# hvak/visual-underwater-slam

Measured on AMD Instinct MI355X. Metric: ORB detect+match frames/sec, higher is better.
Workload: dtype u8

## Files before the change

visual-underwater-slam_amd/csrc/detect.hip:

```cpp
#include "frontend_common.h"
#include "../../include/vus_tiled.h"

namespace {

#ifndef VUS_FAST_WPE
#define VUS_FAST_WPE 1
#endif
#ifndef VUS_FAST_LDS_PAD
#define VUS_FAST_LDS_PAD 0
#endif
#ifdef VUS_FAST_EXIT_AFTER
#define VUS_FAST_EXIT(N) do { if (VUS_FAST_EXIT_AFTER == (N)) return; } while (0)
#else
#define VUS_FAST_EXIT(N)
#endif
#ifdef VUS_FAST_DEBUG_COUNT
__device__ unsigned long long g_fast_dbg[4];
extern "C" int vus_debug_fast_counters(unsigned long long* out, int reset) {
  if (hipMemcpyFromSymbol(out, HIP_SYMBOL(g_fast_dbg), sizeof(g_fast_dbg)) != hipSuccess) return -1;
  if (reset) { unsigned long long z[4] = {0, 0, 0, 0}; if (hipMemcpyToSymbol(HIP_SYMBOL(g_fast_dbg), z, sizeof(z)) != hipSuccess) return -1; }
  return 0;
}
#endif

constexpr int TW = VUS_FAST_TILE_W;
constexpr int TH = VUS_FAST_TILE_H;
constexpr int NTHREADS = 256;
constexpr int IMG_ROWS = TH + 8;
constexpr int IMG_DW = (TW + 16) / 4;
constexpr int SC_ROWS = TH + 2;
constexpr int SC_DW = (TW + 8) / 4;
constexpr int STRIPS = TW / 4;

__device__ __forceinline__ int min3i(int a, int b, int c) { return min(min(a, b), c); }
__device__ __forceinline__ int max3i(int a, int b, int c) { return max(max(a, b), c); }
__device__ __forceinline__ int byte_of(uint32_t w, int i) { return (int)((w >> (8 * i)) & 0xFFu); }

__device__ __forceinline__ int fast_score_bytes(const uint8_t* c, int rb) {
  constexpr int DX[16] = {0, 1, 2, 3, 3, 3, 2, 1, 0, -1, -2, -3, -3, -3, -2, -1};
  constexpr int DY[16] = {-3, -3, -2, -1, 0, 1, 2, 3, 3, 3, 2, 1, 0, -1, -2, -3};
  const int p = c[0];
  int d[16];
#pragma unroll
  for (int k = 0; k < 16; ++k) d[k] = (int)c[DY[k] * rb + DX[k]] - p;
  int mn3[16], mx3[16];
#pragma unroll
  for (int k = 0; k < 16; ++k) {
    mn3[k] = min3i(d[k], d[(k + 1) & 15], d[(k + 2) & 15]);
    mx3[k] = max3i(d[k], d[(k + 1) & 15], d[(k + 2) & 15]);
  }
  int best_bright = -(1 << 20), best_dark = 1 << 20;
#pragma unroll
  for (int k = 0; k < 16; ++k) {
    best_bright = max(best_bright, min3i(mn3[k], mn3[(k + 3) & 15], mn3[(k + 6) & 15]));
    best_dark = min(best_dark, max3i(mx3[k], mx3[(k + 3) & 15], mx3[(k + 6) & 15]));
  }
  return max(best_bright, -best_dark) - 1;
}

constexpr int VUS_CAND_REGIONS = 8;
struct BlurMfmaTable {
  uint64_t h[64];
  uint64_t v[2][64];
};
constexpr BlurMfmaTable make_blur_mfma_table() {
  constexpr int BW[7] = {18, 33, 49, 56, 49, 33, 18};
  BlurMfmaTable t{};
  for (int l = 0; l < 64; ++l) {
    const int g = l >> 4, m = l & 15;
    for (int sl = 0; sl < 8; ++sl) {
      const int d = 8 * g + sl - m - 5;
      if (d >= 0 && d <= 6) t.h[l] |= (uint64_t)BW[d] << (8 * sl);
      const int hrow = sl < 4 ? 4 * g + sl : 16 + 4 * g + (sl - 4);
      for (int nb = 0; nb < 2; ++nb) {
        const int dv = hrow - (16 * nb + m + 1);
        if (dv >= 0 && dv <= 6) t.v[nb][l] |= (uint64_t)BW[dv] << (8 * sl);
      }
    }
  }
  return t;
}
__device__ __attribute__((aligned(16))) const BlurMfmaTable g_blur_mfma_table = make_blur_mfma_table();
typedef int v4i32_t __attribute__((ext_vector_type(4)));

template <bool TILED = false>
__device__ __forceinline__ void blur_tile_mfma(const uint32_t* s_img, uint8_t* __restrict__ blur_out, int n, int H, int W,
                                               int x0, int y0, int tid, int j_first, int j_step) {
  static_assert(IMG_ROWS == 32 && TW % 16 == 0 && (IMG_DW * 4) % 8 == 0, "blur_tile_mfma: K = the 32 staged rows");
  const int l = tid & 63, g = l >> 4, m = l & 15;
  const long bh = (long)g_blur_mfma_table.h[l];
  const long bv[2] = {(long)g_blur_mfma_table.v[0][l], (long)g_blur_mfma_table.v[1][l]};
  const uint8_t* img8 = reinterpret_cast<const uint8_t*>(s_img);
  constexpr unsigned long long SIGN = 0x8080808080808080ull;
  const int j_end = TILED ? min(TW / 16, (W - x0) / 16) : TW / 16;
  bool row_ok[2] = {false, false};
  uint32_t tiled_off[2] = {0u, 0u};
  uint8_t* const tiled_plane = blur_out + (size_t)n * H * W;
  if (TILED) {
    j_first = __builtin_amdgcn_readfirstlane(j_first);
#pragma unroll
    for (int nb = 0; nb < 2; ++nb) {
      const int ly = 16 * nb + m;
      row_ok[nb] = ly < TH && y0 + ly < H;
      tiled_off[nb] = vus_tiled_offset(y0 + ly, x0 + 4 * g, W);
    }
  }
#pragma unroll 1
  for (int j = j_first; j < j_end; j += j_step) {
    v4i32_t ch[2];
#pragma unroll
    for (int mb = 0; mb < 2; ++mb) {
      const unsigned long long a =
          *reinterpret_cast<const unsigned long long*>(img8 + (16 * mb + m) * (IMG_DW * 4) + 16 * j + 8 * g) ^ SIGN;
      const v4i32_t c0 = {32768, 32768, 32768, 32768};
      ch[mb] = __builtin_amdgcn_mfma_i32_16x16x32_i8((long)a, bh, c0, 0, 0, 0);
    }
    uint32_t lo[2], hi[2];
#pragma unroll
    for (int mb = 0; mb < 2; ++mb) {
      const uint32_t t0 = __builtin_amdgcn_perm((uint32_t)ch[mb][1], (uint32_t)ch[mb][0], 0x05010400u);
      const uint32_t t1 = __builtin_amdgcn_perm((uint32_t)ch[mb][3], (uint32_t)ch[mb][2], 0x05010400u);
      lo[mb] = __builtin_amdgcn_perm(t1, t0, 0x05040100u);
      hi[mb] = __builtin_amdgcn_perm(t1, t0, 0x07060302u);
    }
    const long a_lo = (long)((((unsigned long long)lo[1] << 32) | lo[0]) ^ SIGN);
    const long a_hi = (long)((((unsigned long long)hi[1] << 32) | hi[0]) ^ SIGN);
#pragma unroll
    for (int nb = 0; nb < 2; ++nb) {
      const v4i32_t ci = {32768, 32768, 32768, 32768};
      const v4i32_t cl = {65536, 65536, 65536, 65536};
      const v4i32_t chi = __builtin_amdgcn_mfma_i32_16x16x32_i8(a_hi, bv[nb], ci, 0, 0, 0);
      const v4i32_t clo = __builtin_amdgcn_mfma_i32_16x16x32_i8(a_lo, bv[nb], cl, 0, 0, 0);
      uint32_t q[4];
#pragma unroll
      for (int r = 0; r < 4; ++r) q[r] = ((uint32_t)chi[r] << 8) + (uint32_t)clo[r];
      const uint32_t v = __builtin_amdgcn_perm(q[1], q[0], 0x0c0c0602u) | __builtin_amdgcn_perm(q[3], q[2], 0x06020c0cu);
      const int ly = 16 * nb + m, gy = y0 + ly, gx = x0 + 16 * j + 4 * g;
      if (TILED) {
        if (row_ok[nb]) __builtin_memcpy(tiled_plane + (tiled_off[nb] + (uint32_t)(VUS_TILE_BW * VUS_TILE_BH * j)), &v, 4);
      } else if (ly < TH && gy < H) {
        uint8_t* o = blur_out + ((size_t)n * H + gy) * W + gx;
        if (gx + 3 < W) {
          __builtin_memcpy(o, &v, 4);
        } else {
#pragma unroll
          for (int e = 0; e < 4; ++e)
            if (gx + e < W) o[e] = (uint8_t)(v >> (8 * e));
        }
      }
    }
  }
}

template <bool WRITE_SCORE, bool DETECT, bool BLUR, bool HIST = false, bool REGIONS = false, bool TILED = false>
__device__ __forceinline__ void fast_tile_body(
    const uint8_t* __restrict__ img, int H, int W, int pitch, int thr, int border,
    uint8_t* __restrict__ score_out, uint8_t* __restrict__ blur_out,
    uint32_t* __restrict__ cand_keys, int cand_cap, int* __restrict__ cand_count, int* __restrict__ hist,
    int n, int tile, int tiles_x, uint8_t* __restrict__ raw_out = nullptr) {
  static_assert(IMG_ROWS == 32, "the smoothing (blur_tile_mfma) takes the 32 staged rows as its K");
  constexpr bool SCORES = WRITE_SCORE || DETECT;
  constexpr bool LATE_BLUR = BLUR && DETECT && !HIST;
  static_assert(!TILED || LATE_BLUR, "the block-tiled planes are written by the late-smoothing detection launch");

  __shared__ __attribute__((aligned(8))) uint32_t s_img[IMG_ROWS * IMG_DW];
  __shared__ uint32_t s_score[SCORES ? SC_ROWS * SC_DW : 1];
  constexpr int AUX_DW = SCORES ? (IMG_ROWS * IMG_DW + SC_ROWS * SC_DW + 1) / 2 : 2;
  __shared__ uint32_t s_aux[AUX_DW];
  uint16_t* const s_mm = reinterpret_cast<uint16_t*>(s_aux);
  uint16_t* const s_strip = s_mm + IMG_ROWS * IMG_DW;
  __shared__ uint16_t s_work[SCORES ? SC_ROWS * SC_DW * 4 : 2];
  __shared__ int s_nstrip;
  __shared__ int s_cnt, s_base, s_nwork;
  static_assert(IMG_ROWS * IMG_DW >= TW * TH / 4, "candidate list must fit in the image tile");
  static_assert(!LATE_BLUR || AUX_DW >= TW * TH / 4, "candidate list must fit in the strip tables' buffer");
  uint32_t* const s_keys = LATE_BLUR ? s_aux : s_img;

  const int tid = threadIdx.x;
  const int x0 = (tile % tiles_x) * TW, y0 = (tile / tiles_x) * TH;
  const uint8_t* im = img + (size_t)n * H * pitch;

  {
    constexpr int RPP = NTHREADS / IMG_DW;
    const int col = tid % IMG_DW, r0 = tid / IMG_DW;
    const int gx = x0 - 8 + 4 * col;
    const bool fast = gx >= 0 && gx + 3 < W;
    const bool inside = x0 >= 8 && x0 + TW + 8 <= W && y0 >= 4 && y0 + TH + 4 <= H;
    if (r0 < RPP) {
      constexpr int NP = (IMG_ROWS + RPP - 1) / RPP;
      constexpr int LASTP = IMG_ROWS - (NP - 1) * RPP;
      uint32_t v[NP];
      if (inside) {
        const uint32_t off0 = (uint32_t)((y0 - 4 + r0) * pitch + gx);
        const uint32_t step = (uint32_t)(RPP * pitch);
#pragma unroll
        for (int k = 0; k < NP - 1; ++k) __builtin_memcpy(&v[k], im + (off0 + (uint32_t)k * step), 4);
        v[NP - 1] = 0u;
        if (r0 < LASTP) __builtin_memcpy(&v[NP - 1], im + (off0 + (uint32_t)(NP - 1) * step), 4);
      } else {
        const uint8_t* rp[NP];
#pragma unroll
        for (int k = 0; k < NP; ++k) rp[k] = im + (size_t)clampi(y0 - 4 + min(r0 + RPP * k, IMG_ROWS - 1), 0, H - 1) * pitch;
        if (fast) {
#pragma unroll
          for (int k = 0; k < NP; ++k) __builtin_memcpy(&v[k], rp[k] + gx, 4);
        } else {
          const int c0 = clampi(gx, 0, W - 1), c1 = clampi(gx + 1, 0, W - 1), c2 = clampi(gx + 2, 0, W - 1),
                    c3 = clampi(gx + 3, 0, W - 1);
          uint8_t q[NP][4];
#pragma unroll
          for (int k = 0; k < NP; ++k) { q[k][0] = rp[k][c0]; q[k][1] = rp[k][c1]; q[k][2] = rp[k][c2]; q[k][3] = rp[k][c3]; }
#pragma unroll
          for (int k = 0; k < NP; ++k)
            v[k] = (uint32_t)q[k][0] | ((uint32_t)q[k][1] << 8) | ((uint32_t)q[k][2] << 16) | ((uint32_t)q[k][3] << 24);
        }
      }
#pragma unroll
      for (int k = 0; k < NP; ++k) {
        const int row = r0 + RPP * k;
        if (row < IMG_ROWS) {
          s_img[row * IMG_DW + col] = v[k];
          if (SCORES) {
            const int b0 = byte_of(v[k], 0), b1 = byte_of(v[k], 1), b2 = byte_of(v[k], 2), b3 = byte_of(v[k], 3);
            s_mm[row * IMG_DW + col] = (uint16_t)(min(min(b0, b1), min(b2, b3)) | (max(max(b0, b1), max(b2, b3)) << 8));
          }
        }
      }
    }
  }
  if (tid == 0) { s_cnt = 0; s_nwork = 0; s_nstrip = 0; }
  __syncthreads();
  VUS_FAST_EXIT(1);

  if (SCORES) {
    static_assert(STRIPS == 32 && (TH * STRIPS) % NTHREADS == 0, "pass 1a: thread = (row tid >> 5, strip tid & 31)");
    constexpr int S_RPP = NTHREADS / STRIPS;
    constexpr int NMAIN = TH / S_RPP;
    constexpr int NIT = NMAIN + 1;
    static_assert(SC_DW + TH <= 64 && SC_ROWS == TH + 2 && SC_DW == STRIPS + 2, "pass 1a: the ring pass is a row and a column per wave");
    auto strip_test = [&](int sr, int ss, int ci) -> bool {
      const int gy = y0 - 1 + sr, gx = x0 - 4 + 4 * ss;
      if (!((uint32_t)gx < (uint32_t)max(W - 3, 0) && (uint32_t)(gy - 3) < (uint32_t)max(H - 6, 0))) return false;
      const uint8_t* mm8 = reinterpret_cast<const uint8_t*>(s_mm) + 2 * ci;
      const int ma_lo = mm8[0], ma_hi = mm8[1], pmin = mm8[2], pmax = mm8[3], mc_lo = mm8[4], mc_hi = mm8[5];
      const int mn_lo = mm8[2 - 6 * IMG_DW], mn_hi = mm8[3 - 6 * IMG_DW], ms_lo = mm8[2 + 6 * IMG_DW], ms_hi = mm8[3 + 6 * IMG_DW];
      const uint32_t b = s_img[ci + 1];
      const int b0 = byte_of(b, 0), b3 = byte_of(b, 3);
      const int hi = min(max(mn_hi, ms_hi), max3i(ma_hi, mc_hi, max(b0, b3)));
      const int lo = max(min(mn_lo, ms_lo), min3i(ma_lo, mc_lo, min(b0, b3)));
      return hi > pmin + thr || lo < pmax - thr;
    };
    const int sr0 = 1 + (tid >> 5), ss0 = 1 + (tid & 31);
    unsigned long long bal[NIT];
    bool pass[NIT];
    int ent[NIT];
#pragma unroll
    for (int it = 0; it < NMAIN; ++it) {
      const int sr = sr0 + it * S_RPP;
      pass[it] = strip_test(sr, ss0, (sr0 + 3) * IMG_DW + ss0 + it * S_RPP * IMG_DW);
      s_score[sr0 * SC_DW + ss0 + it * S_RPP * SC_DW] = 0u;
      ent[it] = sr * SC_DW + ss0;
      bal[it] = __ballot(pass[it]);
    }
    pass[NMAIN] = false;
    ent[NMAIN] = 0;
    bal[NMAIN] = 0ull;
    const int wv = __builtin_amdgcn_readfirstlane(tid >> 6);
    if (wv < 2) {
      const int l = tid & 63;
      const bool is_row = l < SC_DW;
      const int sr = is_row ? wv * (SC_ROWS - 1) : l - (SC_DW - 1);
      const int ss = is_row ? l : wv * (SC_DW - 1);
      if (l < SC_DW + TH) {
        pass[NMAIN] = strip_test(sr, ss, (sr + 3) * IMG_DW + ss);
        s_score[sr * SC_DW + ss] = 0u;
        ent[NMAIN] = sr * SC_DW + ss;
      }
      bal[NMAIN] = __ballot(pass[NMAIN]);
    }
    int total = 0;
#pragma unroll
    for (int it = 0; it < NIT; ++it) total += __popcll(bal[it]);
    if (total > 0) {
      int base = 0;
      if ((tid & 63) == 0) base = atomicAdd(&s_nstrip, total);
      base = __builtin_amdgcn_readfirstlane(base);
#pragma unroll
      for (int it = 0; it < NIT; ++it) {
        if (pass[it])
          s_strip[base + __builtin_amdgcn_mbcnt_hi((uint32_t)(bal[it] >> 32), __builtin_amdgcn_mbcnt_lo((uint32_t)bal[it], 0))] =
              (uint16_t)ent[it];
        base += __popcll(bal[it]);
      }
    }
    __syncthreads();
    VUS_FAST_EXIT(2);
    const int nstrip = s_nstrip;
#ifdef VUS_FAST_DEBUG_COUNT
    if (tid == 0 && BLUR) { atomicAdd(&g_fast_dbg[0], 1ull); atomicAdd(&g_fast_dbg[1], (unsigned long long)nstrip); }
#endif
    for (int j0 = 0; j0 < nstrip; j0 += NTHREADS) {
      const int j = j0 + tid;
      int mask = 0, idx = 0;
      if (j < nstrip) {
        idx = s_strip[j];
        const int sr = idx / SC_DW, ss = idx - sr * SC_DW;
        const int gx = x0 - 4 + 4 * ss;
        const uint32_t* cp = &s_img[(sr + 3) * IMG_DW + ss];
        const uint32_t a = cp[0], b = cp[1], c = cp[2];
        const uint32_t nn = s_img[sr * IMG_DW + ss + 1], so = s_img[(sr + 6) * IMG_DW + ss + 1];
        const uint32_t wv = __builtin_amdgcn_alignbyte(b, a, 1);
        const uint32_t ev = __builtin_amdgcn_alignbyte(c, b, 3);
        const uint32_t* up = &s_img[(sr + 1) * IMG_DW + ss];
        const uint32_t* dn = &s_img[(sr + 5) * IMG_DW + ss];
        const uint32_t nev = __builtin_amdgcn_alignbyte(up[2], up[1], 2), nwv = __builtin_amdgcn_alignbyte(up[1], up[0], 2);
        const uint32_t sev = __builtin_amdgcn_alignbyte(dn[2], dn[1], 2), swv = __builtin_amdgcn_alignbyte(dn[1], dn[0], 2);
#pragma unroll
        for (int e = 0; e < 4; ++e) {
          const int p = byte_of(b, e);
          const int n_ = byte_of(nn, e), s_ = byte_of(so, e), w_ = byte_of(wv, e), e_ = byte_of(ev, e);
          int hi = min(max(n_, s_), max(e_, w_)), lo = max(min(n_, s_), min(e_, w_));
          const int ne = byte_of(nev, e), sw = byte_of(swv, e), se = byte_of(sev, e), nw = byte_of(nwv, e);
          hi = min3i(hi, max(ne, sw), max(se, nw));
          lo = max3i(lo, min(ne, sw), min(se, nw));
          mask |= (hi > p + thr || lo < p - thr) ? (1 << e) : 0;
        }
        if (gx < 3 || gx + 3 >= W - 3) {
#pragma unroll
          for (int e = 0; e < 4; ++e)
            if (gx + e < 3 || gx + e >= W - 3) mask &= ~(1 << e);
        }
      }
      const int cnt = __popc(mask);
      int incl = cnt;
      incl += __builtin_amdgcn_update_dpp(0, incl, 0x111, 0xf, 0xf, true);
      incl += __builtin_amdgcn_update_dpp(0, incl, 0x112, 0xf, 0xf, true);
      incl += __builtin_amdgcn_update_dpp(0, incl, 0x114, 0xf, 0xe, true);
      incl += __builtin_amdgcn_update_dpp(0, incl, 0x118, 0xf, 0xc, true);
      incl += __builtin_amdgcn_update_dpp(0, incl, 0x142, 0xa, 0xf, true);
      incl += __builtin_amdgcn_update_dpp(0, incl, 0x143, 0xc, 0xf, true);
      const int total = __builtin_amdgcn_readlane(incl, 63);
      int base = 0;
      if ((tid & 63) == 0 && total > 0) base = atomicAdd(&s_nwork, total);
      base = __builtin_amdgcn_readfirstlane(base);
      int pos = base + incl - cnt;
#pragma unroll
      for (int e = 0; e < 4; ++e)
        if (mask & (1 << e)) s_work[pos++] = (uint16_t)(idx * 4 + e);
    }
  }
#ifdef VUS_FAST_DEBUG_COUNT
  __syncthreads();
  if (tid == 0 && BLUR && SCORES) atomicAdd(&g_fast_dbg[2], (unsigned long long)s_nwork);
#endif
  VUS_FAST_EXIT(3);
  if (BLUR && !LATE_BLUR) blur_tile_mfma(s_img, blur_out, n, H, W, x0, y0, tid, tid >> 6, NTHREADS / 64);
  __syncthreads();
  VUS_FAST_EXIT(4);

  if (SCORES) {
    const int nwork = s_nwork;
    uint8_t* score8 = reinterpret_cast<uint8_t*>(s_score);
    for (int j = tid; j < nwork; j += NTHREADS) {
      const int ent = s_work[j];
      const int idx = ent >> 2, e = ent & 3;
      const int sr = idx / SC_DW, ss = idx - sr * SC_DW;
      const int sc = fast_score_bytes(reinterpret_cast<const uint8_t*>(s_img) + (sr + 3) * (4 * IMG_DW) + 4 * (ss + 1) + e, 4 * IMG_DW);
      if (sc >= thr) score8[ent] = (uint8_t)sc;
    }
    __syncthreads();
  }
  VUS_FAST_EXIT(5);

  if (WRITE_SCORE) {
    for (int idx = tid; idx < TH * STRIPS; idx += NTHREADS) {
      const int ly = idx / STRIPS, ls = idx - ly * STRIPS;
      const int gy = y0 + ly, gx = x0 + 4 * ls;
      const uint32_t v = s_score[(ly + 1) * SC_DW + ls + 1];
      if (gy < H) {
        uint8_t* o = score_out + ((size_t)n * H + gy) * W + gx;
#pragma unroll
        for (int e = 0; e < 4; ++e)
          if (gx + e < W) o[e] = (uint8_t)(v >> (8 * e));
      }
    }
  }
  if (DETECT) {
    const int nwork = s_nwork;
    const uint8_t* score8 = reinterpret_cast<const uint8_t*>(s_score);
    for (int j = tid; j < nwork; j += NTHREADS) {
      const int ent = s_work[j];
      const int s = score8[ent];
      if (s == 0) continue;
      const int sr = ent / (4 * SC_DW), sx = ent - sr * (4 * SC_DW);
      const int ly = sr - 1, lx = sx - 4;
      if (ly < 0 || ly >= TH || lx < 0 || lx >= TW) continue;
      const int gy = y0 + ly, gx = x0 + lx;
      if (gy < border || gy >= H - border || gx < border || gx >= W - border) continue;
      const uint8_t* c = score8 + ent;
      constexpr int RB = 4 * SC_DW;
      const int m = max3i(max3i(c[-RB - 1], c[-RB], c[-RB + 1]), max((int)c[-1], (int)c[1]), max3i(c[RB - 1], c[RB], c[RB + 1]));
      if (s > m) {
        if (HIST) {
          atomicAdd(&hist[256 * n + s], 1);
        } else {
          const int p = atomicAdd(&s_cnt, 1);
          s_keys[p] = ((uint32_t)(255 - s) << VUS_KEY_POS_BITS) | (uint32_t)(gy * W + gx);
        }
      }
    }
    if (!HIST) {
      __syncthreads();
      const int cnt = s_cnt;
      const int rcap = cand_cap / VUS_CAND_REGIONS;
      uint32_t* const list = cand_keys + (size_t)n * cand_cap + (REGIONS ? (size_t)(tile & (VUS_CAND_REGIONS - 1)) * rcap : 0);
      int* const counter = REGIONS ? reinterpret_cast<int*>(list) : &cand_count[n];
      if (LATE_BLUR) {
        const bool leader = tid == NTHREADS - 64 && cnt > 0;
        int base = 0;
        if (leader) base = atomicAdd(counter, cnt);
        if (TILED && tid >= NTHREADS - 64) {
          const uint8_t* s8 = reinterpret_cast<const uint8_t*>(s_img);
          uint8_t* const ro = raw_out + (size_t)n * H * W;
          for (int i = tid - (NTHREADS - 64); i < TH * (TW / 16); i += 64) {
            const int ly = i / (TW / 16), cb = i - ly * (TW / 16);
            const int gy = y0 + ly, gx = x0 + 16 * cb;
            if (gy < H && gx < W) {
              const uint8_t* sp = s8 + (ly + 4) * (4 * IMG_DW) + 8 + 16 * cb;
              const uint2 a = *reinterpret_cast<const uint2*>(sp), b = *reinterpret_cast<const uint2*>(sp + 8);
              *reinterpret_cast<uint4*>(ro + vus_tiled_offset(gy, gx, W)) = make_uint4(a.x, a.y, b.x, b.y);
            }
          }
        }
        if (leader) s_base = base;
        if (tid < NTHREADS - 64) blur_tile_mfma<TILED>(s_img, blur_out, n, H, W, x0, y0, tid, tid >> 6, NTHREADS / 64 - 1);
      } else {
        if (tid == 0 && cnt > 0) s_base = atomicAdd(counter, cnt);
      }
      __syncthreads();
      if (cnt > 0) {
        const int base = s_base + (REGIONS ? 1 : 0), lim = REGIONS ? rcap : cand_cap;
        for (int i = tid; i < cnt; i += NTHREADS)
          if (base + i < lim) list[base + i] = s_keys[i];
      }
    }
  }
}

template <bool WRITE_SCORE, bool DETECT, bool BLUR, bool REGIONS = false>
__global__ __launch_bounds__(NTHREADS, VUS_FAST_WPE) void fast_tile_kernel(
    const uint8_t* __restrict__ img, int H, int W, int pitch, int thr, const int* __restrict__ thr_img, int border,
    uint8_t* __restrict__ score_out, uint8_t* __restrict__ blur_out,
    uint32_t* __restrict__ cand_keys, int cand_cap, int* __restrict__ cand_count, int n_img, int tiles_x,
    int tiles_per_img) {
  const int xcd = blockIdx.x & 7, slot = blockIdx.x >> 3;
  const int n = (slot / tiles_per_img) * 8 + xcd;
  if (n >= n_img) return;
  const int tile = slot - (slot / tiles_per_img) * tiles_per_img;
  fast_tile_body<WRITE_SCORE, DETECT, BLUR, false, REGIONS>(img, H, W, pitch, thr_img ? thr_img[n] : thr, border, score_out, blur_out,
                                                            cand_keys, cand_cap, cand_count, nullptr, n, tile, tiles_x);
}

template <bool REGIONS>
__global__ __launch_bounds__(NTHREADS, VUS_FAST_WPE) void fast_tile_tiled_kernel(
    const uint8_t* __restrict__ img, int H, int W, int pitch, const int* __restrict__ thr_img, int border,
    uint8_t* __restrict__ blur_out, uint8_t* __restrict__ raw_out, uint32_t* __restrict__ cand_keys, int cand_cap,
    int* __restrict__ cand_count, int n_img, int tiles_x, int tiles_per_img) {
  const int xcd = blockIdx.x & 7, slot = blockIdx.x >> 3;
  const int n = (slot / tiles_per_img) * 8 + xcd;
  if (n >= n_img) return;
  const int tile = slot - (slot / tiles_per_img) * tiles_per_img;
  fast_tile_body<false, true, true, false, REGIONS, true>(img, H, W, pitch, thr_img[n], border, nullptr, blur_out, cand_keys,
                                                          cand_cap, cand_count, nullptr, n, tile, tiles_x, raw_out);
}

__global__ void cand_region_zero_kernel(uint32_t* __restrict__ cand_keys, int cand_cap, int n_img) {
  const int t = blockIdx.x * blockDim.x + threadIdx.x;
  if (t < n_img * VUS_CAND_REGIONS)
    cand_keys[(size_t)(t / VUS_CAND_REGIONS) * cand_cap + (size_t)(t % VUS_CAND_REGIONS) * (cand_cap / VUS_CAND_REGIONS)] = 0u;
}

__global__ __launch_bounds__(256) void cand_region_merge_kernel(uint32_t* __restrict__ cand_keys, int cand_cap, int* __restrict__ cand_count) {
  __shared__ int s_c[VUS_CAND_REGIONS];
  const int n = blockIdx.x, tid = threadIdx.x;
  const int rcap = cand_cap / VUS_CAND_REGIONS;
  uint32_t* row = cand_keys + (size_t)n * cand_cap;
  if (tid < VUS_CAND_REGIONS) s_c[tid] = (int)row[(size_t)tid * rcap];
  __syncthreads();
  int off = 0;
  long long all = 0;
  bool over = false;
  for (int r = 0; r < VUS_CAND_REGIONS; ++r) {
    const int c = s_c[r], m = min(c, rcap - 1);
    all += c;
    over |= c > rcap - 1;
    const uint32_t* src = row + (size_t)r * rcap + 1;
    for (int i0 = 0; i0 < m; i0 += 256) {
      const int i = i0 + tid;
      const uint32_t v = i < m ? src[i] : 0u;
      __syncthreads();
      if (i < m) row[off + i] = v;
      __syncthreads();
    }
    off += m;
  }
  if (over)
    for (int i = off + tid; i < cand_cap; i += 256) row[i] = VUS_KEY_INVALID;
  if (tid == 0) cand_count[n] = over ? (int)max(all, (long long)cand_cap + 1) : off;
}

__global__ __launch_bounds__(NTHREADS, VUS_FAST_WPE) void fast_sample_kernel(const uint8_t* __restrict__ img, int H, int W, int pitch,
                                                               int thr, int border, int* __restrict__ hist, int n_img,
                                                               int tiles_x, int tiles_per_img, int stride, int n_sampled) {
  const int xcd = blockIdx.x & 7, slot = blockIdx.x >> 3;
  const int n = (slot / n_sampled) * 8 + xcd;
  if (n >= n_img) return;
  const int tile = (slot - (slot / n_sampled) * n_sampled) * stride + stride / 2;
  if (tile >= tiles_per_img) return;
  fast_tile_body<false, true, false, true>(img, H, W, pitch, thr, border, nullptr, nullptr, nullptr, 0, nullptr, hist, n, tile, tiles_x);
}

__global__ __launch_bounds__(256) void fast_pick_threshold_kernel(const int* __restrict__ hist, int n_img, int thr, int floor, int max_kp,
                                                                  long long n_tiles, long long n_sampled, int num, int den,
                                                                  int* __restrict__ thr_img) {
  const int n = blockIdx.x * 4 + (threadIdx.x >> 6), lane = threadIdx.x & 63;
  if (n >= n_img) return;
  const int4 h = reinterpret_cast<const int4*>(hist + 256 * (size_t)n)[lane];
  const int hv[4] = {h.x, h.y, h.z, lane == 63 ? 0 : h.w};
  int above = hv[0] + hv[1] + hv[2] + hv[3];
  int incl = above;
#pragma unroll
  for (int d = 1; d < 64; d <<= 1) {
    const int o = __shfl_down(incl, d);
    if (lane + d < 64) incl += o;
  }
  above = incl - above;
  const long long need = (long long)max_kp * n_sampled * num;
  long long run = above;
  int best = -1;
#pragma unroll
  for (int q = 3; q >= 0; --q) {
    run += hv[q];
    const int t = 4 * lane + q;
    if (best < 0 && t > floor && t <= 254 && run * n_tiles * den >= need) best = t;
  }
#pragma unroll
  for (int d = 32; d >= 1; d >>= 1) best = max(best, __shfl_xor(best, d));
  if (lane == 0) thr_img[n] = best > floor ? best : thr;
}

__global__ __launch_bounds__(1024) void fast_retry_list_kernel(const int* __restrict__ thr_img, int thr, int max_kp, int cand_cap,
                                                               int n_img, int* __restrict__ cand_count,
                                                               int* __restrict__ retry_list, int* __restrict__ retry_count) {
  __shared__ int s_n;
  if (threadIdx.x == 0) s_n = 0;
  __syncthreads();
  for (int n = threadIdx.x; n < n_img; n += 1024)
    if ((thr_img[n] > thr && cand_count[n] < max_kp) || cand_count[n] > cand_cap) {
      retry_list[atomicAdd(&s_n, 1)] = n;
      cand_count[n] = 0;
    }
  __syncthreads();
  if (threadIdx.x == 0) retry_count[0] = s_n;
}

__global__ __launch_bounds__(NTHREADS, VUS_FAST_WPE) void fast_retry_kernel(const uint8_t* __restrict__ img, int H, int W, int pitch, int thr,
                                                              int border, uint32_t* __restrict__ cand_keys, int cand_cap,
                                                              int* __restrict__ cand_count, const int* __restrict__ retry_list,
                                                              const int* __restrict__ retry_count, int tiles_x, int tiles_per_img) {
  const long long items = (long long)retry_count[0] * tiles_per_img;
  for (long long it = blockIdx.x; it < items; it += gridDim.x) {
    const int n = retry_list[it / tiles_per_img], tile = (int)(it % tiles_per_img);
    fast_tile_body<false, true, false>(img, H, W, pitch, thr, border, nullptr, nullptr, cand_keys, cand_cap, cand_count, nullptr, n,
                                       tile, tiles_x);
    __syncthreads();
  }
}

struct TileGrid {
  unsigned blocks;
  int tiles_x, tiles_per_img;
};
TileGrid tile_grid(int n_img, int H, int W) {
  const int tx = (W + TW - 1) / TW, ty = (H + TH - 1) / TH;
  return TileGrid{(unsigned)(((n_img + 7) / 8) * 8 * tx * ty), tx, tx * ty};
}

}

extern "C" int vus_fast_score(const uint8_t* img, int n_img, int H, int W, int pitch, int thr,
                              uint8_t* score_out, void* stream) {
  if (int rc = check_image_args(img, n_img, H, W, pitch)) return rc;
  VUS_REQUIRE(score_out != nullptr, "score_out is null");
  VUS_REQUIRE(thr >= 1 && thr <= 254, "thr=%d out of range [1, 254]", thr);
  if (n_img == 0) return VUS_OK;
  const TileGrid g = tile_grid(n_img, H, W);
  fast_tile_kernel<true, false, false><<<g.blocks, NTHREADS, 0, vus::as_stream(stream)>>>(
      img, H, W, pitch, thr, nullptr, 0, score_out, nullptr, nullptr, 0, nullptr, n_img, g.tiles_x, g.tiles_per_img);
  VUS_CHECK_LAUNCH("fast_score");
  return VUS_OK;
}

extern "C" int vus_blur7(const uint8_t* img, int n_img, int H, int W, int pitch, uint8_t* out, void* stream) {
  if (int rc = check_image_args(img, n_img, H, W, pitch)) return rc;
  VUS_REQUIRE(out != nullptr, "out is null");
  if (n_img == 0) return VUS_OK;
  const TileGrid g = tile_grid(n_img, H, W);
  fast_tile_kernel<false, false, true><<<g.blocks, NTHREADS, 0, vus::as_stream(stream)>>>(
      img, H, W, pitch, 1, nullptr, 0, nullptr, out, nullptr, 0, nullptr, n_img, g.tiles_x, g.tiles_per_img);
  VUS_CHECK_LAUNCH("blur7");
  return VUS_OK;
}

extern "C" int vus_fast_detect(const uint8_t* img, int n_img, int H, int W, int pitch, int thr, int border,
                               uint8_t* blur_out, uint32_t* cand_keys, int cand_cap, int* cand_count,
                               void* stream) {
  if (int rc = check_image_args(img, n_img, H, W, pitch)) return rc;
  VUS_REQUIRE(cand_keys != nullptr && cand_count != nullptr, "candidate buffers are null");
  VUS_REQUIRE(cand_cap >= 1, "cand_cap=%d", cand_cap);
  VUS_REQUIRE(thr >= 1 && thr <= 254, "thr=%d out of range [1, 254]", thr);
  VUS_REQUIRE(border >= 0, "border=%d", border);
  if (n_img == 0) return VUS_OK;
  hipStream_t st = vus::as_stream(stream);
  const TileGrid g = tile_grid(n_img, H, W);
  if (blur_out)
    fast_tile_kernel<false, true, true><<<g.blocks, NTHREADS, 0, st>>>(
        img, H, W, pitch, thr, nullptr, border, nullptr, blur_out, cand_keys, cand_cap, cand_count, n_img, g.tiles_x,
        g.tiles_per_img);
  else
    fast_tile_kernel<false, true, false><<<g.blocks, NTHREADS, 0, st>>>(
        img, H, W, pitch, thr, nullptr, border, nullptr, nullptr, cand_keys, cand_cap, cand_count, n_img, g.tiles_x,
        g.tiles_per_img);
  VUS_CHECK_LAUNCH("fast_detect");
  return VUS_OK;
}

extern "C" int vus_fast_threshold_estimate(const uint8_t* img, int n_img, int H, int W, int pitch, int thr, int border,
                                           int max_kp, int sample_stride, int* hist, int* thr_img, void* stream) {
  if (int rc = check_image_args(img, n_img, H, W, pitch)) return rc;
  VUS_REQUIRE(hist != nullptr && thr_img != nullptr, "null buffer");
  VUS_REQUIRE(thr >= 1 && thr <= 254, "thr=%d out of range [1, 254]", thr);
  VUS_REQUIRE(border >= 0 && max_kp >= 1 && sample_stride >= 1, "border=%d max_kp=%d sample_stride=%d", border, max_kp, sample_stride);
  if (n_img == 0) return VUS_OK;
  hipStream_t st = vus::as_stream(stream);
  const TileGrid g = tile_grid(n_img, H, W);
  const int n_sampled = (g.tiles_per_img - sample_stride / 2 + sample_stride - 1) / sample_stride;
  VUS_CHECK_HIP(hipMemsetAsync(hist, 0, sizeof(int) * 256 * (size_t)n_img, st));
  const int floor = thr > VUS_FAST_SAMPLE_FLOOR ? thr : VUS_FAST_SAMPLE_FLOOR;
  if (n_sampled > 0)
    fast_sample_kernel<<<(unsigned)(((n_img + 7) / 8) * 8 * n_sampled), NTHREADS, 0, st>>>(
        img, H, W, pitch, floor, border, hist, n_img, g.tiles_x, g.tiles_per_img, sample_stride, n_sampled);
  fast_pick_threshold_kernel<<<(n_img + 3) / 4, 256, 0, st>>>(hist, n_img, thr, floor, max_kp, g.tiles_per_img,
                                                                 n_sampled > 0 ? n_sampled : 1, VUS_FAST_MARGIN_NUM,
                                                                 VUS_FAST_MARGIN_DEN, thr_img);
  VUS_CHECK_LAUNCH("fast_threshold_estimate");
  return VUS_OK;
}

extern "C" int vus_fast_detect_adaptive(const uint8_t* img, int n_img, int H, int W, int pitch, const int* thr_img, int border,
                                        uint8_t* blur_out, uint32_t* cand_keys, int cand_cap, int* cand_count, void* stream) {
  if (int rc = check_image_args(img, n_img, H, W, pitch)) return rc;
  VUS_REQUIRE(cand_keys != nullptr && cand_count != nullptr && thr_img != nullptr, "null buffer");
  VUS_REQUIRE(cand_cap >= 1 && border >= 0, "cand_cap=%d border=%d", cand_cap, border);
  if (n_img == 0) return VUS_OK;
  hipStream_t st = vus::as_stream(stream);
  const TileGrid g = tile_grid(n_img, H, W);
  const bool regions = blur_out != nullptr && cand_cap >= 64 * VUS_CAND_REGIONS;
  if (regions) {
    cand_region_zero_kernel<<<(n_img * VUS_CAND_REGIONS + 255) / 256, 256, 0, st>>>(cand_keys, cand_cap, n_img);
    fast_tile_kernel<false, true, true, true><<<g.blocks, NTHREADS, VUS_FAST_LDS_PAD, st>>>(
        img, H, W, pitch, 0, thr_img, border, nullptr, blur_out, cand_keys, cand_cap, cand_count, n_img, g.tiles_x, g.tiles_per_img);
    cand_region_merge_kernel<<<n_img, 256, 0, st>>>(cand_keys, cand_cap, cand_count);
  } else if (blur_out)
    fast_tile_kernel<false, true, true><<<g.blocks, NTHREADS, VUS_FAST_LDS_PAD, st>>>(
        img, H, W, pitch, 0, thr_img, border, nullptr, blur_out, cand_keys, cand_cap, cand_count, n_img, g.tiles_x, g.tiles_per_img);
  else
    fast_tile_kernel<false, true, false><<<g.blocks, NTHREADS, 0, st>>>(
        img, H, W, pitch, 0, thr_img, border, nullptr, nullptr, cand_keys, cand_cap, cand_count, n_img, g.tiles_x, g.tiles_per_img);
  VUS_CHECK_LAUNCH("fast_detect_adaptive");
  return VUS_OK;
}

extern "C" int vus_fast_detect_adaptive_tiled(const uint8_t* img, int n_img, int H, int W, int pitch, const int* thr_img,
                                              int border, uint8_t* blur_tiled, uint8_t* img_tiled, uint32_t* cand_keys,
                                              int cand_cap, int* cand_count, void* stream) {
  if (int rc = check_image_args(img, n_img, H, W, pitch)) return rc;
  if (int rc = check_tiled_args(blur_tiled, img_tiled, H, W)) return rc;
  VUS_REQUIRE(cand_keys != nullptr && cand_count != nullptr && thr_img != nullptr, "null buffer");
  VUS_REQUIRE(cand_cap >= 1 && border >= 0, "cand_cap=%d border=%d", cand_cap, border);
  if (n_img == 0) return VUS_OK;
  hipStream_t st = vus::as_stream(stream);
  const TileGrid g = tile_grid(n_img, H, W);
  static_assert(TW % VUS_TILE_BW == 0 && TH % VUS_TILE_BH == 0, "a detector tile is whole blocks");
  if (cand_cap >= 64 * VUS_CAND_REGIONS) {
    cand_region_zero_kernel<<<(n_img * VUS_CAND_REGIONS + 255) / 256, 256, 0, st>>>(cand_keys, cand_cap, n_img);
    fast_tile_tiled_kernel<true><<<g.blocks, NTHREADS, 0, st>>>(img, H, W, pitch, thr_img, border, blur_tiled, img_tiled,
                                                                cand_keys, cand_cap, cand_count, n_img, g.tiles_x, g.tiles_per_img);
    cand_region_merge_kernel<<<n_img, 256, 0, st>>>(cand_keys, cand_cap, cand_count);
  } else {
    fast_tile_tiled_kernel<false><<<g.blocks, NTHREADS, 0, st>>>(img, H, W, pitch, thr_img, border, blur_tiled, img_tiled,
                                                                 cand_keys, cand_cap, cand_count, n_img, g.tiles_x, g.tiles_per_img);
  }
  VUS_CHECK_LAUNCH("fast_detect_adaptive_tiled");
  return VUS_OK;
}

extern "C" int vus_fast_detect_retry(const uint8_t* img, int n_img, int H, int W, int pitch, int thr, const int* thr_img,
                                     int max_kp, int border, uint32_t* cand_keys, int cand_cap, int* cand_count,
                                     int* retry_list, int* retry_count, void* stream) {
  if (int rc = check_image_args(img, n_img, H, W, pitch)) return rc;
  VUS_REQUIRE(cand_keys && cand_count && thr_img && retry_list && retry_count, "null buffer");
  VUS_REQUIRE(thr >= 1 && thr <= 254 && max_kp >= 1 && cand_cap >= 1 && border >= 0, "thr=%d max_kp=%d cand_cap=%d border=%d", thr,
              max_kp, cand_cap, border);
  if (n_img == 0) return VUS_OK;
  hipStream_t st = vus::as_stream(stream);
  const TileGrid g = tile_grid(n_img, H, W);
  fast_retry_list_kernel<<<1, 1024, 0, st>>>(thr_img, thr, max_kp, cand_cap, n_img, cand_count, retry_list, retry_count);
  int n_cu = 256;
  {
    int dev = 0;
    if (hipGetDevice(&dev) != hipSuccess || hipDeviceGetAttribute(&n_cu, hipDeviceAttributeMultiprocessorCount, dev) != hipSuccess ||
        n_cu < 1)
      n_cu = 256;
  }
  fast_retry_kernel<<<8 * n_cu, NTHREADS, 0, st>>>(img, H, W, pitch, thr, border, cand_keys, cand_cap, cand_count, retry_list,
                                                   retry_count, g.tiles_x, g.tiles_per_img);
  VUS_CHECK_LAUNCH("fast_detect_retry");
  return VUS_OK;
}
```

Measured before the change: 202,200.

## Tag FAST candidates with bright/dark side and score only that side

```diff
diff --git a/visual-underwater-slam_amd/csrc/detect.hip b/visual-underwater-slam_amd/csrc/detect.hip
--- a/visual-underwater-slam_amd/csrc/detect.hip
+++ b/visual-underwater-slam_amd/csrc/detect.hip
@@ -15,10 +15,10 @@
 #define VUS_FAST_EXIT(N)
 #endif
 #ifdef VUS_FAST_DEBUG_COUNT
-__device__ unsigned long long g_fast_dbg[4];
+__device__ unsigned long long g_fast_dbg[5];
 extern "C" int vus_debug_fast_counters(unsigned long long* out, int reset) {
   if (hipMemcpyFromSymbol(out, HIP_SYMBOL(g_fast_dbg), sizeof(g_fast_dbg)) != hipSuccess) return -1;
-  if (reset) { unsigned long long z[4] = {0, 0, 0, 0}; if (hipMemcpyToSymbol(HIP_SYMBOL(g_fast_dbg), z, sizeof(z)) != hipSuccess) return -1; }
+  if (reset) { unsigned long long z[5] = {0, 0, 0, 0, 0}; if (hipMemcpyToSymbol(HIP_SYMBOL(g_fast_dbg), z, sizeof(z)) != hipSuccess) return -1; }
   return 0;
 }
 #endif
@@ -36,13 +36,13 @@
 __device__ __forceinline__ int max3i(int a, int b, int c) { return max(max(a, b), c); }
 __device__ __forceinline__ int byte_of(uint32_t w, int i) { return (int)((w >> (8 * i)) & 0xFFu); }
 
+constexpr int FAST_DX[16] = {0, 1, 2, 3, 3, 3, 2, 1, 0, -1, -2, -3, -3, -3, -2, -1};
+constexpr int FAST_DY[16] = {-3, -3, -2, -1, 0, 1, 2, 3, 3, 3, 2, 1, 0, -1, -2, -3};
 __device__ __forceinline__ int fast_score_bytes(const uint8_t* c, int rb) {
-  constexpr int DX[16] = {0, 1, 2, 3, 3, 3, 2, 1, 0, -1, -2, -3, -3, -3, -2, -1};
-  constexpr int DY[16] = {-3, -3, -2, -1, 0, 1, 2, 3, 3, 3, 2, 1, 0, -1, -2, -3};
   const int p = c[0];
   int d[16];
 #pragma unroll
-  for (int k = 0; k < 16; ++k) d[k] = (int)c[DY[k] * rb + DX[k]] - p;
+  for (int k = 0; k < 16; ++k) d[k] = (int)c[FAST_DY[k] * rb + FAST_DX[k]] - p;
   int mn3[16], mx3[16];
 #pragma unroll
   for (int k = 0; k < 16; ++k) {
@@ -56,6 +56,26 @@
     best_dark = min(best_dark, max3i(mx3[k], mx3[(k + 3) & 15], mx3[(k + 6) & 15]));
   }
   return max(best_bright, -best_dark) - 1;
+}
+
+__device__ __forceinline__ int min3_window(int a, int b, int c) {
+  int r;
+  asm("v_min3_i32 %0, %1, %2, %3" : "=v"(r) : "v"(a), "v"(b), "v"(c));
+  return r;
+}
+__device__ __forceinline__ int fast_score_side(const uint8_t* c, int rb, int flip) {
+  int b[16];
+#pragma unroll
+  for (int k = 0; k < 16; ++k) b[k] = (int)c[FAST_DY[k] * rb + FAST_DX[k]] ^ flip;
+  int w3[16];
+#pragma unroll
+  for (int k = 0; k < 16; ++k) w3[k] = min3_window(b[k], b[(k + 1) & 15], b[(k + 2) & 15]);
+  int w9[16];
+#pragma unroll
+  for (int k = 0; k < 16; ++k) w9[k] = min3_window(w3[k], w3[(k + 3) & 15], w3[(k + 6) & 15]);
+  const int m0 = max3i(w9[0], w9[1], w9[2]), m1 = max3i(w9[3], w9[4], w9[5]), m2 = max3i(w9[6], w9[7], w9[8]);
+  const int m3 = max3i(w9[9], w9[10], w9[11]), m4 = max3i(w9[12], w9[13], w9[14]);
+  return max(max3i(m0, m1, m2), max3i(m3, m4, w9[15])) - ((int)c[0] ^ flip) - 1;
 }
 
 constexpr int VUS_CAND_REGIONS = 8;
@@ -170,6 +190,9 @@
   uint16_t* const s_mm = reinterpret_cast<uint16_t*>(s_aux);
   uint16_t* const s_strip = s_mm + IMG_ROWS * IMG_DW;
   __shared__ uint16_t s_work[SCORES ? SC_ROWS * SC_DW * 4 : 2];
+  constexpr int WORK_SIDE_SHIFT = 14, WORK_INDEX = (1 << 12) - 1;
+  constexpr int WORK_BRIGHT = 1 << WORK_SIDE_SHIFT, WORK_DARK = 2 << WORK_SIDE_SHIFT;
+  static_assert(SC_ROWS * SC_DW * 4 <= WORK_INDEX + 1, "a work-list entry keeps twelve bits for the pixel");
   __shared__ int s_nstrip;
   __shared__ int s_cnt, s_base, s_nwork;
   static_assert(IMG_ROWS * IMG_DW >= TW * TH / 4, "candidate list must fit in the image tile");
@@ -301,7 +324,8 @@
 #endif
     for (int j0 = 0; j0 < nstrip; j0 += NTHREADS) {
       const int j = j0 + tid;
-      int mask = 0, idx = 0;
+      uint32_t side[4] = {0u, 0u, 0u, 0u};
+      int idx = 0;
       if (j < nstrip) {
         idx = s_strip[j];
         const int sr = idx / SC_DW, ss = idx - sr * SC_DW;
@@ -323,15 +347,20 @@
           const int ne = byte_of(nev, e), sw = byte_of(swv, e), se = byte_of(sev, e), nw = byte_of(nwv, e);
           hi = min3i(hi, max(ne, sw), max(se, nw));
           lo = max3i(lo, min(ne, sw), min(se, nw));
-          mask |= (hi > p + thr || lo < p - thr) ? (1 << e) : 0;
+          const uint32_t dark = __builtin_amdgcn_alignbit(e ? side[e - 1] : 0u, (uint32_t)(lo - (p - thr)), 31);
+          side[e] = __builtin_amdgcn_alignbit(dark, (uint32_t)((p + thr) - hi), 31);
         }
         if (gx < 3 || gx + 3 >= W - 3) {
 #pragma unroll
           for (int e = 0; e < 4; ++e)
-            if (gx + e < 3 || gx + e >= W - 3) mask &= ~(1 << e);
+            if (gx + e < 3 || gx + e >= W - 3) {
+              side[e] &= ~3u;
+              side[3] &= ~(3u << (2 * (3 - e)));
+            }
         }
       }
-      const int cnt = __popc(mask);
+      const uint32_t listed = (side[3] | (side[3] >> 1)) & 0x55u;
+      const int cnt = __popc(listed);
       int incl = cnt;
       incl += __builtin_amdgcn_update_dpp(0, incl, 0x111, 0xf, 0xf, true);
       incl += __builtin_amdgcn_update_dpp(0, incl, 0x112, 0xf, 0xf, true);
@@ -346,7 +375,7 @@
       int pos = base + incl - cnt;
 #pragma unroll
       for (int e = 0; e < 4; ++e)
-        if (mask & (1 << e)) s_work[pos++] = (uint16_t)(idx * 4 + e);
+        if (listed & (1u << (2 * (3 - e)))) s_work[pos++] = (uint16_t)(side[e] << WORK_SIDE_SHIFT | (uint32_t)(idx * 4 + e));
     }
   }
 #ifdef VUS_FAST_DEBUG_COUNT
@@ -362,10 +391,21 @@
     const int nwork = s_nwork;
     uint8_t* score8 = reinterpret_cast<uint8_t*>(s_score);
     for (int j = tid; j < nwork; j += NTHREADS) {
-      const int ent = s_work[j];
+      const int went = s_work[j];
+      const int ent = went & WORK_INDEX;
       const int idx = ent >> 2, e = ent & 3;
       const int sr = idx / SC_DW, ss = idx - sr * SC_DW;
-      const int sc = fast_score_bytes(reinterpret_cast<const uint8_t*>(s_img) + (sr + 3) * (4 * IMG_DW) + 4 * (ss + 1) + e, 4 * IMG_DW);
+      const uint8_t* c = reinterpret_cast<const uint8_t*>(s_img) + (sr + 3) * (4 * IMG_DW) + 4 * (ss + 1) + e;
+      int sc;
+      const bool two_sided = __ballot((went & (WORK_BRIGHT | WORK_DARK)) == (WORK_BRIGHT | WORK_DARK)) != 0ull;
+#ifdef VUS_FAST_DEBUG_COUNT
+      if (j == __builtin_amdgcn_readfirstlane(j) && BLUR) { atomicAdd(&g_fast_dbg[3], 1ull); atomicAdd(&g_fast_dbg[4], two_sided ? 1ull : 0ull); }
+#endif
+      if (two_sided) {
+        sc = fast_score_bytes(c, 4 * IMG_DW);
+      } else {
+        sc = fast_score_side(c, 4 * IMG_DW, (went & WORK_BRIGHT) ? 0 : 255);
+      }
       if (sc >= thr) score8[ent] = (uint8_t)sc;
     }
     __syncthreads();
@@ -389,7 +429,7 @@
     const int nwork = s_nwork;
     const uint8_t* score8 = reinterpret_cast<const uint8_t*>(s_score);
     for (int j = tid; j < nwork; j += NTHREADS) {
-      const int ent = s_work[j];
+      const int ent = s_work[j] & WORK_INDEX;
       const int s = score8[ent];
       if (s == 0) continue;
       const int sr = ent / (4 * SC_DW), sx = ent - sr * (4 * SC_DW);
@@ -564,7 +604,7 @@
   if (threadIdx.x == 0) retry_count[0] = s_n;
 }
 
-__global__ __launch_bounds__(NTHREADS, VUS_FAST_WPE) void fast_retry_kernel(const uint8_t* __restrict__ img, int H, int W, int pitch, int thr,
+__global__ __launch_bounds__(NTHREADS, VUS_FAST_WPE > 7 ? VUS_FAST_WPE : 7) void fast_retry_kernel(const uint8_t* __restrict__ img, int H, int W, int pitch, int thr,
                                                               int border, uint32_t* __restrict__ cand_keys, int cand_cap,
                                                               int* __restrict__ cand_count, const int* __restrict__ retry_list,
                                                               const int* __restrict__ retry_count, int tiles_x, int tiles_per_img) {
```

Result: faster. 206,200 (median of 6 runs) (+1.9%).
